# Sahar-E/NeRF-and-DietNeRF

Measured on AMD Instinct MI355X. Metric: rays/sec (coarse+fine) at 256x256, 64 coarse + 128 fine samples, higher is better.
Workload: dtype f16 (3-pass hi/lo split operands, f32 accumulate; fp32-class results)

## Files before the change

### include/nerf_mi355.h

```cpp
#ifndef NERF_MI355_H
#define NERF_MI355_H

#include <stddef.h>
#include <stdint.h>

#ifdef __cplusplus
extern "C" {
#endif

#define NERF_ABI_VERSION 6

enum { NERF_NET_COARSE = 0, NERF_NET_FINE = 1 };
enum { NERF_MEM_HOST = 0, NERF_MEM_DEVICE = 1 };
enum {
    NERF_PRECISION_FP32 = 0,
    NERF_PRECISION_F16X3 = 1,
    NERF_PRECISION_F16 = 2,
    NERF_PRECISION_BF16X3 = 3
};

enum {
    NERF_SAMPLING_LINEAR = 0,
    NERF_SAMPLING_LINDISP = 1
};
// ... 36 lines not shown
int nerf_ctx_set_stream(nerf_ctx* ctx, void* hip_stream);
int nerf_ctx_set_bounds(nerf_ctx* ctx, float near_boundary, float far_boundary);
int nerf_ctx_set_precision(nerf_ctx* ctx, int precision);
int nerf_ctx_set_sampling(nerf_ctx* ctx, int mode);
int nerf_ctx_set_ray_space(nerf_ctx* ctx, int space, float ndc_near_plane);
int nerf_ctx_set_scene_box(nerf_ctx* ctx, const float* lo3, const float* hi3);
int nerf_ctx_set_occupancy_grid(nerf_ctx* ctx, const uint32_t* bits, int32_t R);
int nerf_ctx_get_occupancy_grid(nerf_ctx* ctx, uint32_t* bits, int32_t* R);
int nerf_occupancy_bake(nerf_ctx* ctx, int which, int32_t R, float sigma_threshold, int32_t samples_per_cell, int32_t dilate,
                        uint64_t seed, int64_t* n_occupied);

int nerf_density_lattice(nerf_ctx* ctx, int which, int32_t n, const float* view_dir3, float* sigma, int mem);
int nerf_isosurface(nerf_ctx* ctx, const float* sigma, int32_t n, const float* lo3, const float* hi3, float iso,
                    int64_t* n_vertices, int64_t* n_triangles, int mem);
int nerf_isosurface_fetch(nerf_ctx* ctx, float* vertices, float* normals, int32_t* triangles, int mem);
int nerf_mesh_colors(nerf_ctx* ctx, int which, const float* vertices, const float* normals, int64_t V, float* rgb, int mem);

size_t nerf_blob_size(const nerf_config* cfg);
int nerf_load_weights(nerf_ctx* ctx, int which, const float* blob, size_t n_floats);

int nerf_get_rays_directions(nerf_ctx* ctx, const float* c2w, float fov, int32_t H, int32_t W,
                             float* dirs, int mem);
int nerf_rays_to_ndc(nerf_ctx* ctx, const float* rays_orig, const float* rays_dirs, int64_t N, float fov,
                     float ndc_near_plane, float* out_orig, float* out_dirs, int mem);
int nerf_get_z_values(nerf_ctx* ctx, int64_t N, int32_t S, const float* u, uint64_t seed,
                      int64_t ray_base, float* z, int mem);
int nerf_get_z_values_rays(nerf_ctx* ctx, const float* rays_orig, const float* rays_dirs, int64_t N, int32_t S,
                           const float* u, uint64_t seed, int64_t ray_base, float* z, int mem);
int nerf_ray_box_bounds(nerf_ctx* ctx, const float* rays_orig, const float* rays_dirs, int64_t N, float* bounds,
                        int32_t* narrowed, int mem);
int nerf_ray_occupancy_bounds(nerf_ctx* ctx, const float* rays_orig, const float* rays_dirs, int64_t N, float* bounds,
                              int32_t* state, int mem);
int nerf_ctx_set_sample_culling(nerf_ctx* ctx, int on);
int nerf_ctx_set_train_sample_culling(nerf_ctx* ctx, int on);
int nerf_sample_occupancy(nerf_ctx* ctx, const float* rays_orig, const float* rays_dirs, const float* z, int64_t N, int32_t S,
                          int32_t* keep, int mem);
int nerf_ctx_read_culling(nerf_ctx* ctx, int64_t* samples, int64_t* kept);
int nerf_sample_pdf(nerf_ctx* ctx, const float* weights, const float* z, int64_t N, int32_t S,
                    int32_t Sf, const float* u, uint64_t seed, int64_t ray_base, float* z_new,
                    float* z_merged, int mem);
int nerf_positional_encoding(nerf_ctx* ctx, const float* x, int64_t M, int32_t n_enc,
                             int32_t with_passthrough, float* out, int mem);
int nerf_model_predict(nerf_ctx* ctx, int which, const float* xyz, const float* view_dirs,
                       int64_t M, float* raw, int mem);
int nerf_ray_marching(nerf_ctx* ctx, const float* raw, const float* z, int64_t N, int32_t S,
                      const nerf_outputs* outs, int mem);
int nerf_render_rays(nerf_ctx* ctx, int which, const float* rays_orig, const float* rays_dirs,
                     const float* z, int64_t N, int32_t S, const nerf_outputs* outs, int mem);
int nerf_render(nerf_ctx* ctx, const float* rays_orig, const float* rays_dirs, int64_t N,
                int32_t Sc, int32_t Sf, const float* u_coarse, const float* u_fine, uint64_t seed,
                int64_t ray_base, const nerf_outputs* outs, int mem);
int nerf_render_image(nerf_ctx* ctx, const float* c2w, float fov, int32_t H, int32_t W,
                      int64_t ray_begin, int64_t ray_count, int64_t batch, int32_t Sc, int32_t Sf,
                      const float* u_coarse, const float* u_fine, uint64_t seed,
                      const nerf_outputs* outs, int mem);

int nerf_host_alloc(size_t bytes, void** out);
int nerf_host_free(void* p);

#define NERF_COMM_ID_BYTES 128
int nerf_comm_unique_id(void* id );
int nerf_comm_init(nerf_ctx* ctx, const void* id, int32_t rank, int32_t world);
int nerf_comm_destroy(nerf_ctx* ctx);
int nerf_render_image_sharded(nerf_ctx* ctx, const float* c2w, float field_of_view, int32_t H, int32_t W,
                              int64_t batch, int32_t n_coarse, int32_t n_fine, uint64_t seed,
                              float* rgb , int mem);
// ... 51 lines not shown
```

### nerf_and_dietnerf_amd/_lib.py

```python
from __future__ import annotations

import ctypes as C
import os

_HERE = os.path.dirname(os.path.abspath(__file__))
LIB_PATH = os.environ.get("NERF_MI355_LIB") or os.path.join(_HERE, "lib", "libnerf_mi355.so")

NERF_NET_COARSE, NERF_NET_FINE = 0, 1
NERF_MEM_HOST, NERF_MEM_DEVICE = 0, 1
NERF_PRECISION_FP32, NERF_PRECISION_F16X3, NERF_PRECISION_F16, NERF_PRECISION_BF16X3 = 0, 1, 2, 3
NERF_SAMPLING_LINEAR, NERF_SAMPLING_LINDISP = 0, 1
NERF_RAYS_WORLD, NERF_RAYS_NDC = 0, 1
NERF_ABI_VERSION = 6


class NerfConfig(C.Structure):
    _fields_ = [
        ("n_pos_enc_xyz", C.c_int32), ("n_pos_enc_dir", C.c_int32), ("n_angles", C.c_int32),
        ("hidden_dim", C.c_int32), ("last_hidden_dim", C.c_int32), ("leaky_relu_alpha", C.c_float),
        ("near_boundary", C.c_float), ("far_boundary", C.c_float), ("precision", C.c_int32),
        ("device", C.c_int32),
    ]


# ... 8 lines not shown
                ("rgb", "weights", "cumprod", "alpha", "rgb_samples", "z", "depth")]


_P, _I32, _I64, _U64, _F = C.c_void_p, C.c_int32, C.c_int64, C.c_uint64, C.c_float
SYMBOLS = [
    ("nerf_abi_version", C.c_int, []),
    ("nerf_last_error", C.c_char_p, []),
    ("nerf_ctx_create", C.c_int, [C.POINTER(NerfConfig), C.POINTER(_P)]),
    ("nerf_ctx_destroy", None, [_P]),
    ("nerf_ctx_synchronize", C.c_int, [_P]),
    ("nerf_ctx_set_stream", C.c_int, [_P, _P]),
    ("nerf_ctx_set_bounds", C.c_int, [_P, _F, _F]),
    ("nerf_ctx_set_precision", C.c_int, [_P, C.c_int]),
    ("nerf_ctx_set_sampling", C.c_int, [_P, C.c_int]),
    ("nerf_ctx_set_ray_space", C.c_int, [_P, C.c_int, _F]),
    ("nerf_ctx_set_scene_box", C.c_int, [_P, _P, _P]),
    ("nerf_ctx_set_occupancy_grid", C.c_int, [_P, _P, _I32]),
    ("nerf_ctx_get_occupancy_grid", C.c_int, [_P, _P, _P]),
    ("nerf_occupancy_bake", C.c_int, [_P, C.c_int, _I32, _F, _I32, _I32, _U64, _P]),
    ("nerf_density_lattice", C.c_int, [_P, C.c_int, _I32, _P, _P, C.c_int]),
    ("nerf_isosurface", C.c_int, [_P, _P, _I32, _P, _P, _F, C.POINTER(_I64), C.POINTER(_I64), C.c_int]),
    ("nerf_isosurface_fetch", C.c_int, [_P, _P, _P, _P, C.c_int]),
    ("nerf_mesh_colors", C.c_int, [_P, C.c_int, _P, _P, _I64, _P, C.c_int]),
    ("nerf_blob_size", C.c_size_t, [C.POINTER(NerfConfig)]),
    ("nerf_load_weights", C.c_int, [_P, C.c_int, _P, C.c_size_t]),
    ("nerf_get_rays_directions", C.c_int, [_P, _P, _F, _I32, _I32, _P, C.c_int]),
    ("nerf_rays_to_ndc", C.c_int, [_P, _P, _P, _I64, _F, _F, _P, _P, C.c_int]),
    ("nerf_get_z_values", C.c_int, [_P, _I64, _I32, _P, _U64, _I64, _P, C.c_int]),
    ("nerf_get_z_values_rays", C.c_int, [_P, _P, _P, _I64, _I32, _P, _U64, _I64, _P, C.c_int]),
    ("nerf_ray_box_bounds", C.c_int, [_P, _P, _P, _I64, _P, _P, C.c_int]),
    ("nerf_ray_occupancy_bounds", C.c_int, [_P, _P, _P, _I64, _P, _P, C.c_int]),
    ("nerf_ctx_set_sample_culling", C.c_int, [_P, C.c_int]),
    ("nerf_ctx_set_train_sample_culling", C.c_int, [_P, C.c_int]),
    ("nerf_sample_occupancy", C.c_int, [_P, _P, _P, _P, _I64, _I32, _P, C.c_int]),
    ("nerf_ctx_read_culling", C.c_int, [_P, C.POINTER(_I64), C.POINTER(_I64)]),
    ("nerf_ctx_read_culling_timing", C.c_int, [_P, C.POINTER(C.c_double), C.POINTER(_I64)]),
    ("nerf_sample_pdf", C.c_int, [_P, _P, _P, _I64, _I32, _I32, _P, _U64, _I64, _P, _P, C.c_int]),
    ("nerf_positional_encoding", C.c_int, [_P, _P, _I64, _I32, _I32, _P, C.c_int]),
    ("nerf_model_predict", C.c_int, [_P, C.c_int, _P, _P, _I64, _P, C.c_int]),
    ("nerf_ray_marching", C.c_int, [_P, _P, _P, _I64, _I32, C.POINTER(NerfOutputs), C.c_int]),
    ("nerf_render_rays", C.c_int, [_P, C.c_int, _P, _P, _P, _I64, _I32, C.POINTER(NerfOutputs), C.c_int]),
    ("nerf_render", C.c_int, [_P, _P, _P, _I64, _I32, _I32, _P, _P, _U64, _I64, C.POINTER(NerfOutputs), C.c_int]),
    ("nerf_render_image", C.c_int, [_P, _P, _F, _I32, _I32, _I64, _I64, _I64, _I32, _I32, _P, _P, _U64,
                                    C.POINTER(NerfOutputs), C.c_int]),
    ("nerf_host_alloc", C.c_int, [C.c_size_t, C.POINTER(_P)]),
    ("nerf_host_free", C.c_int, [_P]),
    ("nerf_comm_unique_id", C.c_int, [_P]),
    ("nerf_comm_init", C.c_int, [_P, _P, _I32, _I32]),
    ("nerf_comm_destroy", C.c_int, [_P]),
    ("nerf_render_image_sharded", C.c_int, [_P, _P, _F, _I32, _I32, _I64, _I32, _I32, _U64, _P, C.c_int]),
    ("nerf_render_image_sharded_outputs", C.c_int, [_P, _P, _F, _I32, _I32, _I64, _I32, _I32, _U64, C.POINTER(NerfOutputs),
                                                    C.c_int]),
    ("nerf_ctx_read_nonfinite", C.c_int, [_P, C.POINTER(_I64)]),
    ("nerf_train_begin", C.c_int, [_P, C.POINTER(NerfTrainConfig)]),
    ("nerf_train_end", C.c_int, [_P]),
    ("nerf_train_set_learning_rate", C.c_int, [_P, _F]),
    ("nerf_train_set_loss_weights", C.c_int, [_P, _F, _F]),
    ("nerf_train_loss_scale", C.c_int, [_P, C.POINTER(C.c_float), C.POINTER(_I64), C.POINTER(_I64)]),
    ("nerf_train_read_metric_sums", C.c_int, [_P, C.POINTER(C.c_double), C.POINTER(_I64)]),
    ("nerf_train_step", C.c_int, [_P, _P, _P, _P, _I64, _I32, _I32, _P, _P, _U64, _P, C.c_int]),
    ("nerf_train_gradients", C.c_int, [_P, _P, _P, _P, _I64, _I32, _I32, _P, _P, _U64, _P, _P, _P, C.c_int]),
    ("nerf_train_apply", C.c_int, [_P, _P, _P, C.c_int]),
    ("nerf_train_render_gradients", C.c_int, [_P, _P, _P, _P, _I64, _I32, _I32, _P, _P, _U64, _I64, _I32, _P, _P, _P,
                                              C.c_int]),
    ("nerf_train_render_forward", C.c_int, [_P, _I32, _P, _P, _I64, _I32, _I32, _P, _P, _U64, _I64, _P, C.c_int]),
    ("nerf_train_render_backward", C.c_int, [_P, _I32, _P, _I32, _P, _P, C.c_int]),
# ... 42 lines not shown
```

### nerf_and_dietnerf_amd/csrc/mlp_f16x3.hip

```cpp
#include "mlp_f16_frag.h"

#include <math.h>
#include <string.h>

#if defined(NERF_BF16) && NERF_PE_LX == 5
namespace nerf::bf16 {
#elif defined(NERF_BF16)
namespace nerf::bf16::wide {
#elif NERF_PE_LX == 5
namespace nerf {
#else
namespace nerf::wide {
#endif

#ifdef NERF_BF16
typedef __bf16 e8 __attribute__((ext_vector_type(8)));
typedef __bf16 bf2 __attribute__((ext_vector_type(2)));
#define NERF_MFMA_E16 __builtin_amdgcn_mfma_f32_32x32x16_bf16
__device__ __forceinline__ void split_e(float y, float& hi_f, float& lo_f) {
    hi_f = __uint_as_float(__float_as_uint(y) & 0xFFFF0000u);
    lo_f = y - hi_f;
}
__device__ __forceinline__ uint32_t pack_hi(float a, float b) {
    return __builtin_amdgcn_perm(__float_as_uint(b), __float_as_uint(a), 0x07060302u);
// ... 300 lines not shown
    for (int e = 0; e < 8; e += 2) {
        if constexpr (FAST) {
            hi[e >> 1] = pack_h2(v[e], v[e + 1]);
            lo[e >> 1] = 0u;
            continue;
        }
        float h0, l0, h1, l1;
        split_e(v[e], h0, l0);
        split_e(v[e + 1], h1, l1);
        hi[e >> 1] = pack_hi(h0, h1);
        lo[e >> 1] = pack_lo(l0, l1);
    }
}

template <bool FAST, bool STASH = false, bool XYZ = false, bool SIGONLY = false>
__device__ __forceinline__ void mlp_f16_body(const MlpArgs& a) {
    static_assert(!SIGONLY || (!FAST && !STASH && !XYZ), "the sigma-only variant is a render kernel of the 3-pass network");
#if defined(NERF_BF16) || NERF_PE_LX != 5
    constexpr bool kPPBuild = false;
#else
    constexpr bool kPPBuild = true;
#endif
    constexpr bool kPP = kPPBuild && !FAST && !STASH && !XYZ;
    extern __shared__ __attribute__((aligned(16))) char smem[];
    const int tid = threadIdx.x;
    const int lane = tid & 63;
    const int wave = __builtin_amdgcn_readfirstlane(tid >> 6);
    const int j = lane & 31;
    const int h = lane >> 5;
    const uint32_t lane16 = kLdsRing + lane * 16;
    uint32_t cb_h = kLdsConst + h * 16;
    asm volatile("" : "+v"(cb_h));

    const long long ntiles = (a.M + 127) / 128;
    if ((long long)blockIdx.x >= ntiles) return;

    for (int i = tid; i < (XYZ ? kXConstFloats : kHConstFloats) / 4; i += 256) {
        const bool sig = SIGONLY && i >= kHConstBias8 / 4 && i < (kHConstBias8 + 32) / 4;
        reinterpret_cast<f32x4*>(smem + kLdsConst)[i] =
            reinterpret_cast<const f32x4*>(a.wconst)[sig ? i + (kHConstBiasSig - kHConstBias8) / 4 : i];
    }

    Pipe p;
    p.ck = 0;
    p.src_next = 0;
    p.n_chunks = XYZ ? (FAST ? kXFStreamChunks : kXStreamChunks) : SIGONLY ? kHStreamChunksSig : (FAST ? kFStreamChunks : kHStreamChunks);
    p.wbase = reinterpret_cast<const char*>(a.wstream);
    p.voff = wave * (kHCQ / 4 * kQuadBytes) + lane * 16;
    p.wave_lds = wave * (kHCQ / 4 * kQuadBytes);
    __syncthreads();
#pragma unroll
    for (int c = 0; c < kHRing - 1; ++c) {
        p.cur_src = p.wbase + (size_t)p.src_next * kHChunkBytes;
        p.cur_dst = kLdsRing + c * kHChunkBytes + p.wave_lds;
        p.src_next += 1;
#pragma unroll
        for (int j = 0; j < kHCQ / 4; ++j) dma_piece(p.cur_src, p.voff + j * kQuadBytes, p.cur_dst + j * kQuadBytes);
    }
    asm volatile("s_waitcnt vmcnt(%0)" ::"n"((kHCQ / 4) * (kHRing - 2)) : "memory");
    __builtin_amdgcn_s_barrier();
    asm volatile("" ::: "memory");

    frag4 xh[16], xl[16], nh[kPP ? 16 : 14], nl[kPP ? 16 : 14], peh[kHStepsPE], pel[kHStepsPE], dh[2], dl[2];
    f32x16 accs[4];
    float xc[64];
    float sigma_raw = 0.f;

    unsigned long long t0 = 0, t1 = 0, acc_t[8] = {0, 0, 0, 0, 0, 0, 0, 0};
    (void)t0; (void)t1; (void)acc_t;
    for (long long tile = blockIdx.x; tile < ntiles; tile += gridDim.x) {
        STAMP(t0);
        const long long m = tile * 128 + wave * 32 + j;
        const bool valid = m < a.M;
        const long long mm = valid ? m : a.M - 1;
        float px, py, pz, dx, dy, dz;
        if (a.mode == 0) {
            const long long ray = mm / a.S;
            const f32x4 o = *reinterpret_cast<const f32x4*>(a.in_a + ray * 4);
            const f32x4 d = *reinterpret_cast<const f32x4*>(a.in_b + ray * 4);
            const float zz = a.z[mm];
            px = __fadd_rn(o[0], __fmul_rn(d[0], zz));
            py = __fadd_rn(o[1], __fmul_rn(d[1], zz));
            pz = __fadd_rn(o[2], __fmul_rn(d[2], zz));
            dx = d[0]; dy = d[1]; dz = d[2];
        } else {
            px = a.in_a[mm * 3 + 0]; py = a.in_a[mm * 3 + 1]; pz = a.in_a[mm * 3 + 2];
            if constexpr (XYZ) { dx = dy = dz = 0.f; }
            else { dx = a.in_b[mm * 3 + 0]; dy = a.in_b[mm * 3 + 1]; dz = a.in_b[mm * 3 + 2]; }
        }
        const float kPi = 3.1415927410125732f;
        float pv[8 * kHStepsPE];
#pragma unroll
        for (int c = 0; c < 3; ++c) {
            const float v = c == 0 ? px : c == 1 ? py : pz;
            if constexpr (FAST) {
                sin_ladder_fp16_modes<kPeLx>(v * kPi, h, &pv[c * kPeLx]);
            } else {
#pragma unroll
                for (int k = 0; k < kPeLx; ++k) pv[c * kPeLx + k] = sin_shifted(v * (kPi * (float)(1 << k)), h);
            }
        }
        if constexpr (kPeLx == 5) {
            pv[15] = h ? 0.f : px; pv[16] = h ? 0.f : py; pv[17] = h ? 0.f : pz;
#pragma unroll
            for (int i = 18; i < 24; ++i) pv[i] = 0.f;
        } else {
            static_assert(kPeLx == 10, "the wide-PE layout holds exactly 10 octaves");
            pv[30] = h ? pz : px; pv[31] = h ? 0.f : py;
        }
#pragma unroll
// ... 120 lines not shown
                    o0 = fmaf(w0[e], x, o0);
                    o1 = fmaf(w1[e], x, o1);
                    o2 = fmaf(w2[e], x, o2);
                }
            }
        }
        o0 += __shfl_xor(o0, 32);
        o1 += __shfl_xor(o1, 32);
        o2 += __shfl_xor(o2, 32);
        const f32x4 bh = lds_read4(kLdsConst + (XYZ ? kXConstBHead : kHConstBHead) * 4);
        if (valid && h == 0) {
            f32x4 out;
            out[0] = o0 + bh[0]; out[1] = o1 + bh[1]; out[2] = o2 + bh[2]; out[3] = sigma_raw;
            *reinterpret_cast<f32x4*>(a.raw + m * 4) = out;
            const float chk = out[0] + out[1] + out[2] + out[3];
            if (a.nonfinite && !(fabsf(chk) <= 3.0e38f)) atomicAdd(a.nonfinite, 1ull);
        }
        STAMP(t0); acc_t[5] += t0 - t1; acc_t[6] += 1;
    }
#ifdef NERF_STAMPS
    if (blockIdx.x == 0 && tid == 0)
        for (int i = 0; i < 8; ++i) g_stamps_h[i] = acc_t[i];
#endif
    asm volatile("s_waitcnt vmcnt(0)" ::: "memory");
}

#ifdef NERF_BF16
__global__ __launch_bounds__(256, 1) void mlp_bf16x3_kernel(const MlpArgs a) { mlp_f16_body<false>(a); }
__global__ __launch_bounds__(256, 1) void mlp_bf16x3_xyz_kernel(const MlpArgs a) { mlp_f16_body<false, false, true>(a); }
#if NERF_PE_LX == 5
__global__ __launch_bounds__(256, 1) void mlp_bf16x3_sig_kernel(const MlpArgs a) { mlp_f16_body<false, false, false, true>(a); }
#endif

static int bf_grid(const MlpArgs& a, int num_cus) {
    const long long ntiles = (a.M + 127) / 128;
    return (int)(ntiles < (long long)num_cus ? ntiles : (long long)num_cus);
}
void launch_mlp_bf16x3(const MlpArgs& a, int num_cus, hipStream_t stream, bool xyz_only) {
    if (a.M <= 0) return;
    if (xyz_only) hipLaunchKernelGGL(mlp_bf16x3_xyz_kernel, dim3(bf_grid(a, num_cus)), dim3(256), kLdsTotal, stream, a);
    else hipLaunchKernelGGL(mlp_bf16x3_kernel, dim3(bf_grid(a, num_cus)), dim3(256), kLdsTotal, stream, a);
}
#if NERF_PE_LX == 5
void launch_mlp_bf16x3_sig(const MlpArgs& a, int num_cus, hipStream_t stream) {
    if (a.M <= 0) return;
    hipLaunchKernelGGL(mlp_bf16x3_sig_kernel, dim3(bf_grid(a, num_cus)), dim3(256), kLdsTotal, stream, a);
}
#endif
void mlp_bf16x3_set_attributes() {
    (void)hipFuncSetAttribute(reinterpret_cast<const void*>(mlp_bf16x3_kernel),
                              hipFuncAttributeMaxDynamicSharedMemorySize, kLdsTotal);
    (void)hipFuncSetAttribute(reinterpret_cast<const void*>(mlp_bf16x3_xyz_kernel),
                              hipFuncAttributeMaxDynamicSharedMemorySize, kLdsTotal);
#if NERF_PE_LX == 5
    (void)hipFuncSetAttribute(reinterpret_cast<const void*>(mlp_bf16x3_sig_kernel),
                              hipFuncAttributeMaxDynamicSharedMemorySize, kLdsTotal);
#endif
}
#else
__global__ __launch_bounds__(256, 1) void mlp_f16x3_kernel(const MlpArgs a) { mlp_f16_body<false>(a); }
__global__ __launch_bounds__(256, 1) void mlp_f16_kernel(const MlpArgs a) { mlp_f16_body<true>(a); }
__global__ __launch_bounds__(256, 1) void mlp_f16x3_stash_kernel(const MlpArgs a) { mlp_f16_body<false, true>(a); }
__global__ __launch_bounds__(256, 1) void mlp_f16_stash_kernel(const MlpArgs a) { mlp_f16_body<true, true>(a); }
__global__ __launch_bounds__(256, 1) void mlp_f16x3_xyz_kernel(const MlpArgs a) { mlp_f16_body<false, false, true>(a); }
#if NERF_PE_LX == 5
__global__ __launch_bounds__(256, 1) void mlp_f16x3_sig_kernel(const MlpArgs a) { mlp_f16_body<false, false, false, true>(a); }
#endif
__global__ __launch_bounds__(256, 1) void mlp_f16_xyz_kernel(const MlpArgs a) { mlp_f16_body<true, false, true>(a); }
__global__ __launch_bounds__(256, 1) void mlp_f16x3_xyz_stash_kernel(const MlpArgs a) { mlp_f16_body<false, true, true>(a); }
__global__ __launch_bounds__(256, 1) void mlp_f16_xyz_stash_kernel(const MlpArgs a) { mlp_f16_body<true, true, true>(a); }

void launch_mlp_f16x3_stash(const MlpArgs& a, int num_cus, hipStream_t stream, bool single_pass, bool xyz_only) {
    if (a.M <= 0) return;
    const long long ntiles = (a.M + 127) / 128;
    const int grid = (int)(ntiles < (long long)num_cus ? ntiles : (long long)num_cus);
    if (xyz_only) {
        if (single_pass) hipLaunchKernelGGL(mlp_f16_xyz_stash_kernel, dim3(grid), dim3(256), kLdsTotal, stream, a);
        else hipLaunchKernelGGL(mlp_f16x3_xyz_stash_kernel, dim3(grid), dim3(256), kLdsTotal, stream, a);
        return;
    }
    if (single_pass) hipLaunchKernelGGL(mlp_f16_stash_kernel, dim3(grid), dim3(256), kLdsTotal, stream, a);
    else hipLaunchKernelGGL(mlp_f16x3_stash_kernel, dim3(grid), dim3(256), kLdsTotal, stream, a);
}

void launch_mlp_f16x3(const MlpArgs& a, int num_cus, hipStream_t stream, bool single_pass, bool xyz_only) {
    if (a.M <= 0) return;
    const long long ntiles = (a.M + 127) / 128;
    const int grid = (int)(ntiles < (long long)num_cus ? ntiles : (long long)num_cus);
    if (xyz_only) {
        if (single_pass) hipLaunchKernelGGL(mlp_f16_xyz_kernel, dim3(grid), dim3(256), kLdsTotal, stream, a);
        else hipLaunchKernelGGL(mlp_f16x3_xyz_kernel, dim3(grid), dim3(256), kLdsTotal, stream, a);
        return;
    }
    if (single_pass) hipLaunchKernelGGL(mlp_f16_kernel, dim3(grid), dim3(256), kLdsTotal, stream, a);
    else hipLaunchKernelGGL(mlp_f16x3_kernel, dim3(grid), dim3(256), kLdsTotal, stream, a);
}

#if NERF_PE_LX == 5
void launch_mlp_f16x3_sig(const MlpArgs& a, int num_cus, hipStream_t stream) {
    if (a.M <= 0) return;
    const long long ntiles = (a.M + 127) / 128;
    const int grid = (int)(ntiles < (long long)num_cus ? ntiles : (long long)num_cus);
    hipLaunchKernelGGL(mlp_f16x3_sig_kernel, dim3(grid), dim3(256), kLdsTotal, stream, a);
}
#endif

#if defined(NERF_STAMPS) && NERF_PE_LX == 5
extern "C" void nerf_debug_read_stamps_h(unsigned long long* out) {
    (void)hipDeviceSynchronize();
    (void)hipMemcpyFromSymbol(out, HIP_SYMBOL(g_stamps_h), sizeof(unsigned long long) * 16);
}
#endif

void mlp_f16x3_set_attributes() {
    (void)hipFuncSetAttribute(reinterpret_cast<const void*>(mlp_f16x3_kernel),
                              hipFuncAttributeMaxDynamicSharedMemorySize, kLdsTotal);
    (void)hipFuncSetAttribute(reinterpret_cast<const void*>(mlp_f16_kernel),
                              hipFuncAttributeMaxDynamicSharedMemorySize, kLdsTotal);
    (void)hipFuncSetAttribute(reinterpret_cast<const void*>(mlp_f16x3_stash_kernel),
                              hipFuncAttributeMaxDynamicSharedMemorySize, kLdsTotal);
    (void)hipFuncSetAttribute(reinterpret_cast<const void*>(mlp_f16_stash_kernel),
                              hipFuncAttributeMaxDynamicSharedMemorySize, kLdsTotal);
    (void)hipFuncSetAttribute(reinterpret_cast<const void*>(mlp_f16x3_xyz_kernel),
                              hipFuncAttributeMaxDynamicSharedMemorySize, kLdsTotal);
    (void)hipFuncSetAttribute(reinterpret_cast<const void*>(mlp_f16_xyz_kernel),
                              hipFuncAttributeMaxDynamicSharedMemorySize, kLdsTotal);
    (void)hipFuncSetAttribute(reinterpret_cast<const void*>(mlp_f16x3_xyz_stash_kernel),
                              hipFuncAttributeMaxDynamicSharedMemorySize, kLdsTotal);
    (void)hipFuncSetAttribute(reinterpret_cast<const void*>(mlp_f16_xyz_stash_kernel),
                              hipFuncAttributeMaxDynamicSharedMemorySize, kLdsTotal);
#if NERF_PE_LX == 5
    (void)hipFuncSetAttribute(reinterpret_cast<const void*>(mlp_f16x3_sig_kernel),
                              hipFuncAttributeMaxDynamicSharedMemorySize, kLdsTotal);
#endif
// ... 269 lines not shown
```

### nerf_and_dietnerf_amd/csrc/nerf_api.hip

```cpp
#include "../../include/nerf_mi355.h"

#include <stdarg.h>
#include <stdio.h>
#include <stdlib.h>
#include <string.h>

#include <algorithm>
#include <cmath>
#include <string>
#include <vector>

#include "nerf_ctx.h"

using namespace nerf;

thread_local std::string g_err;

namespace nerf {

int fail(const char* fmt, ...) {
    char buf[512];
    va_list ap;
    va_start(ap, fmt);
    vsnprintf(buf, sizeof buf, fmt, ap);
// ... 175 lines not shown
        else if (wide_pe) *k = {kBf16x3, kConst16, [](const MlpArgs& a, int n, hipStream_t s, bool x) { bf16::wide::launch_mlp_bf16x3(a, n, s, x); }, false};
        else *k = {kBf16x3, kConst16, [](const MlpArgs& a, int n, hipStream_t s, bool x) { bf16::launch_mlp_bf16x3(a, n, s, x); }, false};
        return 0;
    }
    fail("unknown precision %d", precision);
    return 2;
}

int check_cfg(const nerf_config* cfg) {
    if (!cfg) return fail("nerf_config is NULL");
    if (cfg->n_angles != 2 && cfg->n_angles != 1 && cfg->n_angles != 0)
        return fail("n_angles_for_model should be 1 or 2.");
    if (cfg->n_pos_enc_xyz < 1 || cfg->n_pos_enc_xyz > kLxWide || cfg->n_pos_enc_dir < 1 || cfg->n_pos_enc_dir > kLd ||
        cfg->hidden_dim != kHidden || cfg->last_hidden_dim != kLast)
        return fail("supported networks: n_pos_enc_dim_xyz 1..%d, n_pos_enc_view_dir 1..%d, hidden %d, last hidden %d "
                    "(got %d %d %d %d)", kLxWide, kLd, kHidden, kLast, cfg->n_pos_enc_xyz, cfg->n_pos_enc_dir, cfg->hidden_dim,
                    cfg->last_hidden_dim);
    RenderKernel k;
    if (pick_render_kernel(*cfg, cfg->precision, false, &k) == 2)
        return fail("unknown precision %d (NERF_PRECISION_FP32 = 0, NERF_PRECISION_F16X3 = 1, NERF_PRECISION_F16 = 2, "
                    "NERF_PRECISION_BF16X3 = 3)", cfg->precision);
    return 0;
}

int run_mlp(nerf_ctx* c, int which, const RenderKernel& k, const float* in_a, const float* in_b, const float* z, float* raw,
            long long M, int S, int mode) {
    if (!c->net[which].loaded) return fail("network %d has no weights loaded", which);
    if (int r = train_flush_weights(c, which)) return r;
    MlpArgs a{};
    a.wstream = (const float*)c->net[which].stream[k.stream];
    a.wconst = c->net[which].cst[k.cst];
    if (!a.wstream || !a.wconst) return fail("internal: network %d keeps no stream of kind %d", which, (int)k.stream);
    a.in_a = in_a; a.in_b = in_b; a.z = z; a.raw = raw; a.M = M; a.S = S; a.mode = mode;
    a.nonfinite = c->nonfinite;
    a.alpha = c->cfg.leaky_relu_alpha;
    hipEvent_t e0 = nullptr, e1 = nullptr;
    if (c->timing) {
        if (c->ev_used == c->ev_pool.size()) {
            hipEvent_t x, y;
            HIP_OK(hipEventCreate(&x));
            HIP_OK(hipEventCreate(&y));
            c->ev_pool.emplace_back(x, y);
        }
        e0 = c->ev_pool[c->ev_used].first; e1 = c->ev_pool[c->ev_used].second;
        c->ev_used++;
        c->timed_rows += M;
        HIP_OK(hipEventRecord(e0, c->stream));
    }
    k.launch(a, c->num_cus, c->stream, c->cfg.n_angles == 0);
    if (c->timing) HIP_OK(hipEventRecord(e1, c->stream));
    HIP_OK(hipGetLastError());
    return 0;
}

struct OutSizes { size_t per_ray[7]; };
OutSizes out_sizes(int S) {
    OutSizes o;
    o.per_ray[0] = 3; o.per_ray[1] = S; o.per_ray[2] = S; o.per_ray[3] = S; o.per_ray[4] = 3 * (size_t)S;
    o.per_ray[5] = S; o.per_ray[6] = 1;
    return o;
}
float** out_ptrs(nerf_outputs& o, int i) {
    switch (i) {
        case 0: return &o.rgb; case 1: return &o.weights; case 2: return &o.cumprod; case 3: return &o.alpha;
        case 4: return &o.rgb_samples; case 5: return &o.z; default: return &o.depth;
    }
// ... 581 lines not shown
        if (narrowed) HIP_OK(hipMemcpyAsync(narrowed, dn, (size_t)N * 4, hipMemcpyDeviceToHost, c->stream));
        HIP_OK(hipStreamSynchronize(c->stream));
    }
    return 0;
}

int nerf_ray_occupancy_bounds(nerf_ctx* c, const float* rays_orig, const float* rays_dirs, int64_t N, float* bounds,
                              int32_t* state, int mem) {
    ENTER(c);
    if (!rays_orig || !rays_dirs || !bounds) return fail("NULL argument");
    if (N < 0) return fail("bad shape N=%lld", (long long)N);
    if (!c->box_on || c->grid_R == 0) return fail("no occupancy grid is set (nerf_ctx_set_occupancy_grid, nerf_occupancy_bake)");
    const float *o = rays_orig, *d = rays_dirs;
    float* db = bounds;
    int32_t* ds = state;
    if (mem == NERF_MEM_HOST) {
        if (int r = h2d(c, c->b_orig, rays_orig, (size_t)N * 16)) return r;
        if (int r = h2d(c, c->b_dirs, rays_dirs, (size_t)N * 16)) return r;
        if (int r = ensure(c, c->b_in0, (size_t)N * 8)) return r;
        o = (const float*)c->b_orig.p; d = (const float*)c->b_dirs.p; db = (float*)c->b_in0.p;
        if (state) { if (int r = ensure(c, c->b_in1, (size_t)N * 4)) return r; ds = (int32_t*)c->b_in1.p; }
    }
    launch_ray_grid_bounds(c->box, c->cfg.near_boundary, c->cfg.far_boundary, (const uint32_t*)c->b_grid[c->grid_cur].p, c->grid_R,
                           o, d, N, db, ds, c->stream);
    HIP_OK(hipGetLastError());
    if (mem == NERF_MEM_HOST) {
        HIP_OK(hipMemcpyAsync(bounds, db, (size_t)N * 8, hipMemcpyDeviceToHost, c->stream));
        if (state) HIP_OK(hipMemcpyAsync(state, ds, (size_t)N * 4, hipMemcpyDeviceToHost, c->stream));
        HIP_OK(hipStreamSynchronize(c->stream));
    }
    return 0;
}

int nerf_ctx_set_sample_culling(nerf_ctx* c, int on) {
    if (!c) return fail("ctx is NULL");
    c->cull_on = on != 0;
    return 0;
}

int nerf_ctx_set_train_sample_culling(nerf_ctx* c, int on) {
    if (!c) return fail("ctx is NULL");
    c->train_cull_on = on != 0;
    return 0;
}

int nerf_sample_occupancy(nerf_ctx* c, const float* rays_orig, const float* rays_dirs, const float* z, int64_t N, int32_t S,
                          int32_t* keep, int mem) {
    ENTER(c);
    if (!rays_orig || !rays_dirs || !z || !keep) return fail("NULL argument");
    if (N < 0 || S <= 0) return fail("bad shape N=%lld S=%d", (long long)N, S);
    if (!c->box_on || c->grid_R == 0) return fail("no occupancy grid is set (nerf_ctx_set_occupancy_grid, nerf_occupancy_bake)");
    if (N == 0) return 0;
    const float *o = rays_orig, *d = rays_dirs, *dz = z;
    int32_t* dk = keep;
    if (mem == NERF_MEM_HOST) {
        if (int r = h2d(c, c->b_orig, rays_orig, (size_t)N * 16)) return r;
        if (int r = h2d(c, c->b_dirs, rays_dirs, (size_t)N * 16)) return r;
        if (int r = h2d(c, c->b_zc, z, (size_t)N * S * 4)) return r;
        if (int r = ensure(c, c->b_in0, (size_t)N * S * 4)) return r;
        o = (const float*)c->b_orig.p; d = (const float*)c->b_dirs.p; dz = (const float*)c->b_zc.p; dk = (int32_t*)c->b_in0.p;
    }
    launch_sample_keep(c->box, (const uint32_t*)c->b_grid[c->grid_cur].p, c->grid_R, o, d, dz, N, S, nullptr, dk, c->stream);
    HIP_OK(hipGetLastError());
    if (mem == NERF_MEM_HOST) {
        HIP_OK(hipMemcpyAsync(keep, dk, (size_t)N * S * 4, hipMemcpyDeviceToHost, c->stream));
        HIP_OK(hipStreamSynchronize(c->stream));
// ... 283 lines not shown
```

### nerf_and_dietnerf_amd/csrc/nerf_ctx.h

```cpp
#pragma once
#include "../../include/nerf_mi355.h"

#include <string>
#include <utility>
#include <vector>

#include "nerf_kernels.h"

namespace nerf {

int fail(const char* fmt, ...);

#define HIP_OK(expr)                                                                                    \
    do {                                                                                                \
        hipError_t e__ = (expr);                                                                        \
        if (e__ != hipSuccess) return nerf::fail("%s failed: %s (%s:%d)", #expr, hipGetErrorString(e__), \
                                                 __FILE__, __LINE__);                                   \
    } while (0)

struct DevBuf {
    void* p = nullptr;
    size_t cap = 0;
};

struct NetWeights {
    void* stream[kStreamKinds] = {};
    float* cst[kConstBlocks] = {};
    bool loaded = false;
    std::vector<float> host_blob;
};

struct TrainState;
struct CommState;

}

struct nerf_ctx {
    nerf_config cfg;
    int sampling = NERF_SAMPLING_LINEAR;
    int ray_space = NERF_RAYS_WORLD;
    float ndc_near_plane = 1.0f;
    bool box_on = false;
    nerf::SceneBox box = {};
    int grid_R = 0;
    int grid_cur = 0;
    nerf::DevBuf b_grid[2];
    nerf::DevBuf b_gbounds, b_gstate;
    bool cull_on = false;
    bool train_cull_on = false;
    long long cull_samples = 0, cull_kept = 0;
    uint32_t* cull_rows = nullptr;
    nerf::DevBuf b_cmask, b_cfirst, b_csums;
    nerf::DevBuf b_cxyz, b_cdirs, b_craw;
    std::vector<hipEvent_t> cull_ev;
    size_t cull_ev_used = 0;
    bool mesh_on = false;
    long long mesh_V = 0, mesh_T = 0;
    nerf::DevBuf b_mesh_v, b_mesh_n, b_mesh_t;
    nerf::DevBuf b_mesh_sigma, b_mesh_mask, b_mesh_first, b_mesh_count, b_mesh_tfirst, b_mesh_sums;
    nerf::DevBuf b_lattice;
    int num_cus = 0;
    hipStream_t own_stream = nullptr;
    hipStream_t stream = nullptr;
    hipStream_t copy_stream = nullptr;
    std::vector<hipEvent_t> copy_ev;
    nerf::NetWeights net[2];
    nerf::DevBuf b_orig, b_dirs, b_zc, b_zf, b_raw, b_wc, b_u0, b_u1, b_in0, b_in1, b_in2;
    nerf::DevBuf b_out[7];
    bool timing = false;
    std::vector<std::pair<hipEvent_t, hipEvent_t>> ev_pool;
    size_t ev_used = 0;
    long long timed_rows = 0;
    unsigned long long* nonfinite = nullptr;
    nerf::TrainState* train = nullptr;
    nerf::CommState* comm = nullptr;
};

namespace nerf {

int ensure(nerf_ctx* c, DevBuf& b, size_t bytes);
// ... 17 lines not shown
```

### nerf_and_dietnerf_amd/csrc/nerf_kernels.h

```cpp
#pragma once
#include <hip/hip_runtime.h>
#include <stdint.h>

namespace nerf {

constexpr int kLx = 5;
constexpr int kLd = 4;
constexpr int kHidden = 256;
constexpr int kLast = 128;
constexpr int kXyzDim = 3 + 6 * kLx;
constexpr int kDirDim = 6 * kLd;
size_t blob_floats(int lx, int ld, int n_angles);
void blob_expand_index(int lx, int ld, int n_angles, int32_t* idx, int layout_lx = kLx);

constexpr int kQuadBytes = 1024;
constexpr int kChunkQuads = 16;
constexpr int kChunkBytes = kQuadBytes * kChunkQuads;
constexpr int kRingChunks = 8;
constexpr int kRingBytes = kChunkBytes * kRingChunks;

constexpr int kQpuPE = 5;
constexpr int kQpuHid = 32;
constexpr int kQpuSkip = kQpuPE + kQpuHid;
constexpr int kQpuLast = kQpuHid + 3;
constexpr int kChunksPE = (8 * kQpuPE + 15) / 16;
constexpr int kChunksHid = (8 * kQpuHid) / 16;
constexpr int kChunksSkip = (8 * kQpuSkip + 15) / 16;
constexpr int kChunksLast = (4 * kQpuLast + 15) / 16;
constexpr int kStreamChunks = kChunksPE + 3 * kChunksHid + kChunksSkip + 3 * kChunksHid + kChunksLast;
constexpr size_t kStreamBytes = size_t(kStreamChunks) * kChunkBytes;
constexpr size_t kStreamBytesXyzF32 = size_t(142) * kChunkBytes;
constexpr size_t kStreamBytesF16 = size_t(66) * 32 * kQuadBytes;
constexpr size_t kStreamBytesF16Hi = size_t(33) * 32 * kQuadBytes;
constexpr size_t kStreamBytesF16Sig = size_t(62) * 32 * kQuadBytes;
constexpr size_t kStreamBytesF16Xyz = size_t(73) * 32 * kQuadBytes;
constexpr size_t kStreamBytesF16HiXyz = size_t(37) * 32 * kQuadBytes;

constexpr int kConstBias = 0;
constexpr int kConstBias8 = 2048;
constexpr int kConstWrgb = 2176;
constexpr int kConstBHead = 2560;
constexpr int kConstWsigH = 2564;
constexpr int kConstWsigD = 2820;
constexpr int kConstFloats = 3136;
constexpr int kConstBytes = kConstFloats * 4;

constexpr int kLdsRing = 0;
constexpr int kLdsConst = kRingBytes;
constexpr int kLdsTotal = kRingBytes + kConstBytes;

struct MlpArgs {
    const float* wstream;
    const float* wconst;
    const float* in_a;
    const float* in_b;
    const float* z;
    float* raw;
    unsigned long long* nonfinite;
    long long M;
    int S;
    int mode;
    float alpha;
    float* st_ptr[10];
    int st_ld[10];
    uint32_t* mask_ptr[10];
    int diag_wrap;
};

void launch_mlp_fp32(const MlpArgs& a, int num_cus, hipStream_t stream, bool xyz_only = false);
void mlp_fp32_set_attributes();
void pack_weights_fp32(const float* blob, int n_angles, float* stream_out , float* const_out );

void launch_mlp_f16x3(const MlpArgs& a, int num_cus, hipStream_t stream, bool single_pass = false, bool xyz_only = false);
void launch_mlp_f16x3_stash(const MlpArgs& a, int num_cus, hipStream_t stream, bool single_pass = false, bool xyz_only = false);
size_t f16_stream_bytes(int n_angles, bool hi_only);
void build_f16x3_gather(int n_angles, bool hi_only, int32_t* stream_idx ,
                        int32_t* const_idx );
void launch_repack_f16x3(const float* blob, const int32_t* stream_idx, void* stream, const int32_t* const_idx, float* cst,
                         size_t stream_bytes, hipStream_t s);
void mlp_f16x3_set_attributes();
void pack_weights_f16x3(const float* blob, int n_angles, void* stream_out, float* const_out );
void pack_weights_f16(const float* blob, int n_angles, void* stream_out, float* const_out );
void launch_mlp_f16x3_sig(const MlpArgs& a, int num_cus, hipStream_t stream);
void pack_weights_f16x3_sig(const float* blob, int n_angles, void* stream_out, float* const_out );
void build_f16x3_sig_gather(int n_angles, int32_t* stream_idx );

constexpr int kLxWide = 10;
namespace wide {
void launch_mlp_f16x3(const MlpArgs& a, int num_cus, hipStream_t stream, bool single_pass = false, bool xyz_only = false);
void launch_mlp_f16x3_stash(const MlpArgs& a, int num_cus, hipStream_t stream, bool single_pass = false, bool xyz_only = false);
void build_f16x3_gather(int n_angles, bool hi_only, int32_t* stream_idx, int32_t* const_idx);
void mlp_f16x3_set_attributes();
void pack_weights_f16x3(const float* blob, int n_angles, void* stream_out, float* const_out);
void pack_weights_f16(const float* blob, int n_angles, void* stream_out, float* const_out);
}
namespace bf16 {
void launch_mlp_bf16x3(const MlpArgs& a, int num_cus, hipStream_t stream, bool xyz_only = false);
void launch_mlp_bf16x3_sig(const MlpArgs& a, int num_cus, hipStream_t stream);
void mlp_bf16x3_set_attributes();
// ... 111 lines not shown
```

### nerf_and_dietnerf_amd/render.py

```python
from __future__ import annotations

import ctypes as C
from typing import Dict, List, Optional, Sequence, Tuple

import numpy as np

from . import _lib
from ._lib import (NerfTrainConfig, NERF_MEM_DEVICE, NERF_MEM_HOST, NERF_NET_COARSE, NERF_NET_FINE, NERF_PRECISION_F16X3,
                   NERF_PRECISION_FP32, NerfConfig, NerfOutputs)

N_RENDER_SAMPLES_FINE = "n_render_samples_fine"
N_RENDER_SAMPLES_COARSE = "n_render_samples_coarse"
N_POS_ENC_DIM_XYZ = "n_pos_enc_dim_xyz"
N_POS_ENC_VIEW_DIR = "n_pos_enc_view_dir"
N_ANGLES_FOR_MODEL = "n_angles_for_model"
LEAKY_RELU_ALPHA = "leaky_relu_alpha"
HIDDEN_LAYER_DIM = "hidden_layer_dim"
LAST_HIDDEN_LAYER_DIM = "last_hidden_layer_dim"
N_RAYS_IN_BATCH_RENDER = "n_rays_in_batch_render"
N_RAYS_IN_BATCH_TRAIN = "n_rays_in_batch_train"
LINDISP = "lindisp"
USE_NDC = "use_ndc"
NDC_NEAR_PLANE = "ndc_near_plane"
SCENE_BOX = "scene_box"
# ... 368 lines not shown
            pt = triangles.ctypes.data
        _lib.check(self.lib.nerf_isosurface_fetch(self.h, pvx, pn, pt, arr.mem))
        return vertices, triangles, nrm

    def mesh_colors(self, which, vertices, normals):
        arr = self._arrays(vertices, normals)
        v = int(vertices.shape[0])
        pvx, pn = arr.inp(vertices, (v, 3)), arr.inp(normals, (v, 3))

        def run():
            out, p = arr.out((v, 3))
            _lib.check(self.lib.nerf_mesh_colors(self.h, int(which), pvx, pn, v, p, arr.mem))
            return out
        return self._auto_call(run, arr.mem)

    def ray_occupancy_bounds(self, rays_orig, rays_dirs):
        arr = self._arrays(rays_orig, rays_dirs)
        n = int(rays_orig.shape[0])
        po, pd = arr.inp(rays_orig, (n, 4)), arr.inp(rays_dirs, (n, 4))
        bounds, pb = arr.out((n, 2))
        if arr.torch is not None:
            state = arr.torch.empty((n,), dtype=arr.torch.int32, device=arr.device)
            ps = state.data_ptr()
        else:
            state = np.empty((n,), np.int32)
            ps = state.ctypes.data
        _lib.check(self.lib.nerf_ray_occupancy_bounds(self.h, po, pd, n, pb, ps, arr.mem))
        return bounds, state

    def set_sample_culling(self, on) -> None:
        _lib.check(self.lib.nerf_ctx_set_sample_culling(self.h, int(bool(on))))
        self.sample_culling = bool(on)

    def set_train_sample_culling(self, on) -> None:
        _lib.check(self.lib.nerf_ctx_set_train_sample_culling(self.h, int(bool(on))))
        self._train_sample_culling = bool(on)

    @property
    def train_sample_culling(self) -> bool:
        return self._train_sample_culling

    def sample_occupancy(self, rays_orig, rays_dirs, z_values):
        arr = self._arrays(rays_orig, rays_dirs, z_values)
        n, s = int(z_values.shape[0]), int(z_values.shape[1])
        po, pd, pz = arr.inp(rays_orig, (n, 4)), arr.inp(rays_dirs, (n, 4)), arr.inp(z_values, (n, s))
        if arr.torch is not None:
            keep = arr.torch.empty((n, s), dtype=arr.torch.int32, device=arr.device)
            pk = keep.data_ptr()
        else:
            keep = np.empty((n, s), np.int32)
            pk = keep.ctypes.data
        _lib.check(self.lib.nerf_sample_occupancy(self.h, po, pd, pz, n, s, pk, arr.mem))
        return keep

    def read_culling(self) -> Tuple[int, int]:
        samples, kept = C.c_int64(), C.c_int64()
        _lib.check(self.lib.nerf_ctx_read_culling(self.h, C.byref(samples), C.byref(kept)))
        return samples.value, kept.value

    def read_culling_timing(self) -> Tuple[Tuple[float, float, float, float], int]:
        ms, n = (C.c_double * 4)(), C.c_int64()
        _lib.check(self.lib.nerf_ctx_read_culling_timing(self.h, ms, C.byref(n)))
        return tuple(ms), n.value

    def ray_box_bounds(self, rays_orig, rays_dirs):
        arr = self._arrays(rays_orig, rays_dirs)
# ... 700 lines not shown
```

Before: 1.748 million.

## Add ray-block row ordering for coarse MLP tiles

Adds an alternative mapping of MLP rows to wave lanes in which each 32-lane wave holds 32 different rays at the same sample index instead of 32 consecutive samples along one ray. It is on by default for the coarse network and off for the fine one, and exposed through a new API setter. The intent is likely better coherence or load balance, for example similar view-direction and branch behaviour per wave, or better access patterns for ray inputs. The cost is extra index arithmetic per tile and more scattered z and raw accesses, since rows are strided by S.

```diff
diff --git a/include/nerf_mi355.h b/include/nerf_mi355.h
--- a/include/nerf_mi355.h
+++ b/include/nerf_mi355.h
@@ -92,6 +92,7 @@
 int nerf_ray_occupancy_bounds(nerf_ctx* ctx, const float* rays_orig, const float* rays_dirs, int64_t N, float* bounds,
                               int32_t* state, int mem);
 int nerf_ctx_set_sample_culling(nerf_ctx* ctx, int on);
+int nerf_ctx_set_row_order(nerf_ctx* ctx, int coarse, int fine);
 int nerf_ctx_set_train_sample_culling(nerf_ctx* ctx, int on);
 int nerf_sample_occupancy(nerf_ctx* ctx, const float* rays_orig, const float* rays_dirs, const float* z, int64_t N, int32_t S,
                           int32_t* keep, int mem);
diff --git a/nerf_and_dietnerf_amd/_lib.py b/nerf_and_dietnerf_amd/_lib.py
--- a/nerf_and_dietnerf_amd/_lib.py
+++ b/nerf_and_dietnerf_amd/_lib.py
@@ -64,6 +64,7 @@
     ("nerf_ray_occupancy_bounds", C.c_int, [_P, _P, _P, _I64, _P, _P, C.c_int]),
     ("nerf_ctx_set_sample_culling", C.c_int, [_P, C.c_int]),
     ("nerf_ctx_set_train_sample_culling", C.c_int, [_P, C.c_int]),
+    ("nerf_ctx_set_row_order", C.c_int, [_P, C.c_int, C.c_int]),
     ("nerf_sample_occupancy", C.c_int, [_P, _P, _P, _P, _I64, _I32, _P, C.c_int]),
     ("nerf_ctx_read_culling", C.c_int, [_P, C.POINTER(_I64), C.POINTER(_I64)]),
     ("nerf_ctx_read_culling_timing", C.c_int, [_P, C.POINTER(C.c_double), C.POINTER(_I64)]),
diff --git a/nerf_and_dietnerf_amd/csrc/mlp_f16x3.hip b/nerf_and_dietnerf_amd/csrc/mlp_f16x3.hip
--- a/nerf_and_dietnerf_amd/csrc/mlp_f16x3.hip
+++ b/nerf_and_dietnerf_amd/csrc/mlp_f16x3.hip
@@ -356,7 +356,9 @@
     uint32_t cb_h = kLdsConst + h * 16;
     asm volatile("" : "+v"(cb_h));
 
-    const long long ntiles = (a.M + 127) / 128;
+    constexpr bool kOrders = !FAST && !STASH && !XYZ;
+    const bool order1 = kOrders && a.order == kRowOrderRayBlocks;
+    const long long ntiles = row_order_tiles(order1 ? kRowOrderRayBlocks : kRowOrderRay, a.N, a.S, a.M);
     if ((long long)blockIdx.x >= ntiles) return;
 
     for (int i = tid; i < (XYZ ? kXConstFloats : kHConstFloats) / 4; i += 256) {
@@ -394,12 +396,19 @@
     (void)t0; (void)t1; (void)acc_t;
     for (long long tile = blockIdx.x; tile < ntiles; tile += gridDim.x) {
         STAMP(t0);
-        const long long m = tile * 128 + wave * 32 + j;
-        const bool valid = m < a.M;
-        const long long mm = valid ? m : a.M - 1;
+        long long m = tile * 128 + wave * 32 + j;
+        bool valid = m < a.M;
+        long long mm = valid ? m : a.M - 1;
+        long long ray1 = 0;
+        if (order1) {
+            const RowSlot rs = row_order_lane(kRowOrderRayBlocks, (unsigned)tile * 4u + (unsigned)wave, j, a.N, a.S);
+            valid = rs.valid;
+            ray1 = rs.ray;
+            m = mm = rs.ray * a.S + rs.s;
+        }
         float px, py, pz, dx, dy, dz;
         if (a.mode == 0) {
-            const long long ray = mm / a.S;
+            const long long ray = order1 ? ray1 : mm / a.S;
             const f32x4 o = *reinterpret_cast<const f32x4*>(a.in_a + ray * 4);
             const f32x4 d = *reinterpret_cast<const f32x4*>(a.in_b + ray * 4);
             const float zz = a.z[mm];
@@ -586,13 +595,13 @@
 __global__ __launch_bounds__(256, 1) void mlp_bf16x3_sig_kernel(const MlpArgs a) { mlp_f16_body<false, false, false, true>(a); }
 #endif
 
-static int bf_grid(const MlpArgs& a, int num_cus) {
-    const long long ntiles = (a.M + 127) / 128;
+static int bf_grid(const MlpArgs& a, int num_cus, bool orders = true) {
+    const long long ntiles = row_order_tiles(orders ? a.order : kRowOrderRay, a.N, a.S, a.M);
     return (int)(ntiles < (long long)num_cus ? ntiles : (long long)num_cus);
 }
 void launch_mlp_bf16x3(const MlpArgs& a, int num_cus, hipStream_t stream, bool xyz_only) {
     if (a.M <= 0) return;
-    if (xyz_only) hipLaunchKernelGGL(mlp_bf16x3_xyz_kernel, dim3(bf_grid(a, num_cus)), dim3(256), kLdsTotal, stream, a);
+    if (xyz_only) hipLaunchKernelGGL(mlp_bf16x3_xyz_kernel, dim3(bf_grid(a, num_cus, false)), dim3(256), kLdsTotal, stream, a);
     else hipLaunchKernelGGL(mlp_bf16x3_kernel, dim3(bf_grid(a, num_cus)), dim3(256), kLdsTotal, stream, a);
 }
 #if NERF_PE_LX == 5
@@ -639,7 +648,7 @@
 
 void launch_mlp_f16x3(const MlpArgs& a, int num_cus, hipStream_t stream, bool single_pass, bool xyz_only) {
     if (a.M <= 0) return;
-    const long long ntiles = (a.M + 127) / 128;
+    const long long ntiles = row_order_tiles(single_pass || xyz_only ? kRowOrderRay : a.order, a.N, a.S, a.M);
     const int grid = (int)(ntiles < (long long)num_cus ? ntiles : (long long)num_cus);
     if (xyz_only) {
         if (single_pass) hipLaunchKernelGGL(mlp_f16_xyz_kernel, dim3(grid), dim3(256), kLdsTotal, stream, a);
@@ -653,7 +662,7 @@
 #if NERF_PE_LX == 5
 void launch_mlp_f16x3_sig(const MlpArgs& a, int num_cus, hipStream_t stream) {
     if (a.M <= 0) return;
-    const long long ntiles = (a.M + 127) / 128;
+    const long long ntiles = row_order_tiles(a.order, a.N, a.S, a.M);
     const int grid = (int)(ntiles < (long long)num_cus ? ntiles : (long long)num_cus);
     hipLaunchKernelGGL(mlp_f16x3_sig_kernel, dim3(grid), dim3(256), kLdsTotal, stream, a);
 }
diff --git a/nerf_and_dietnerf_amd/csrc/nerf_api.hip b/nerf_and_dietnerf_amd/csrc/nerf_api.hip
--- a/nerf_and_dietnerf_amd/csrc/nerf_api.hip
+++ b/nerf_and_dietnerf_amd/csrc/nerf_api.hip
@@ -231,6 +231,10 @@
     a.wconst = c->net[which].cst[k.cst];
     if (!a.wstream || !a.wconst) return fail("internal: network %d keeps no stream of kind %d", which, (int)k.stream);
     a.in_a = in_a; a.in_b = in_b; a.z = z; a.raw = raw; a.M = M; a.S = S; a.mode = mode;
+    a.N = mode == 0 ? M / S : M;
+    const bool ordered = mode == 0 && c->cfg.n_angles != 0 &&
+                         (k.stream == kF16x3 || k.stream == kBf16x3 || k.stream == kF16x3Sig || k.stream == kBf16x3Sig);
+    a.order = ordered && row_order_slots(c->row_order[which], a.N, S, M) < kRowOrderMaxSlots ? c->row_order[which] : kRowOrderRay;
     a.nonfinite = c->nonfinite;
     a.alpha = c->cfg.leaky_relu_alpha;
     hipEvent_t e0 = nullptr, e1 = nullptr;
@@ -878,6 +882,16 @@
     return 0;
 }
 
+int nerf_ctx_set_row_order(nerf_ctx* c, int coarse, int fine) {
+    if (!c) return fail("ctx is NULL");
+    const int want[2] = {coarse, fine}, dflt[2] = {kDefaultRowOrderCoarse, kDefaultRowOrderFine};
+    for (int w = 0; w < 2; ++w)
+        if (want[w] < -1 || want[w] > kRowOrderRayBlocks)
+            return fail("row order %d of network %d: 0 (along the ray), 1 (ray blocks) or -1 (the library's default)", want[w], w);
+    for (int w = 0; w < 2; ++w) c->row_order[w] = want[w] < 0 ? dflt[w] : want[w];
+    return 0;
+}
+
 int nerf_ctx_set_sample_culling(nerf_ctx* c, int on) {
     if (!c) return fail("ctx is NULL");
     c->cull_on = on != 0;
diff --git a/nerf_and_dietnerf_amd/csrc/nerf_ctx.h b/nerf_and_dietnerf_amd/csrc/nerf_ctx.h
--- a/nerf_and_dietnerf_amd/csrc/nerf_ctx.h
+++ b/nerf_and_dietnerf_amd/csrc/nerf_ctx.h
@@ -30,6 +30,8 @@
     std::vector<float> host_blob;
 };
 
+constexpr int kDefaultRowOrderCoarse = kRowOrderRayBlocks, kDefaultRowOrderFine = kRowOrderRay;
+
 struct TrainState;
 struct CommState;
 
@@ -46,6 +48,7 @@
     int grid_cur = 0;
     nerf::DevBuf b_grid[2];
     nerf::DevBuf b_gbounds, b_gstate;
+    int row_order[2] = {nerf::kDefaultRowOrderCoarse, nerf::kDefaultRowOrderFine};
     bool cull_on = false;
     bool train_cull_on = false;
     long long cull_samples = 0, cull_kept = 0;
diff --git a/nerf_and_dietnerf_amd/csrc/nerf_kernels.h b/nerf_and_dietnerf_amd/csrc/nerf_kernels.h
--- a/nerf_and_dietnerf_amd/csrc/nerf_kernels.h
+++ b/nerf_and_dietnerf_amd/csrc/nerf_kernels.h
@@ -1,6 +1,8 @@
 #pragma once
 #include <hip/hip_runtime.h>
 #include <stdint.h>
+
+#include "row_order.h"
 
 namespace nerf {
 
@@ -65,6 +67,8 @@
     int st_ld[10];
     uint32_t* mask_ptr[10];
     int diag_wrap;
+    int order;
+    long long N;
 };
 
 void launch_mlp_fp32(const MlpArgs& a, int num_cus, hipStream_t stream, bool xyz_only = false);
diff --git a/nerf_and_dietnerf_amd/csrc/row_order.h b/nerf_and_dietnerf_amd/csrc/row_order.h
--- /dev/null
+++ b/nerf_and_dietnerf_amd/csrc/row_order.h
@@ -0,0 +1,38 @@
+#pragma once
+#if defined(__HIPCC__)
+#define NERF_RO_HD __host__ __device__
+#else
+#define NERF_RO_HD
+#endif
+
+namespace nerf {
+
+constexpr int kRowOrderRay = 0, kRowOrderRayBlocks = 1;
+
+NERF_RO_HD inline long long row_order_slots(int order, long long N, int S, long long M) {
+    return order == kRowOrderRayBlocks ? ((N + 31) / 32) * (long long)S : (M + 31) / 32;
+}
+NERF_RO_HD inline long long row_order_tiles(int order, long long N, int S, long long M) {
+    return order == kRowOrderRayBlocks ? (row_order_slots(order, N, S, M) + 3) / 4 : (M + 127) / 128;
+}
+
+struct RowSlot {
+    long long ray;
+    int s;
+    bool valid;
+};
+NERF_RO_HD inline RowSlot row_order_lane(int order, unsigned q, int j, long long N, int S) {
+    if (order == kRowOrderRayBlocks) {
+        const unsigned g = q / (unsigned)S, s = q - g * (unsigned)S;
+        const long long r = 32ll * g + j;
+        const bool valid = r < N;
+        return {valid ? r : N - 1, (int)s, valid};
+    }
+    const long long M = N * (long long)S, m = 32ll * q + j;
+    const bool valid = m < M;
+    const long long mm = valid ? m : M - 1;
+    return {mm / S, (int)(mm % S), valid};
+}
+constexpr long long kRowOrderMaxSlots = 1ll << 31;
+
+}
diff --git a/nerf_and_dietnerf_amd/render.py b/nerf_and_dietnerf_amd/render.py
--- a/nerf_and_dietnerf_amd/render.py
+++ b/nerf_and_dietnerf_amd/render.py
@@ -424,6 +424,9 @@
         _lib.check(self.lib.nerf_ctx_set_sample_culling(self.h, int(bool(on))))
         self.sample_culling = bool(on)
 
+    def set_row_order(self, coarse: int = -1, fine: int = -1) -> None:
+        _lib.check(self.lib.nerf_ctx_set_row_order(self.h, int(coarse), int(fine)))
+
     def set_train_sample_culling(self, on) -> None:
         _lib.check(self.lib.nerf_ctx_set_train_sample_culling(self.h, int(bool(on))))
         self._train_sample_culling = bool(on)
```

Measured after the change: 1.753 million, median of 6. Within noise of the previous version (+0.3%).
